# MahanFathi/iLQG-MuJoCo

Hardware: AMD Instinct MI355X
Metric: iLQR iterations/sec (FD+backward+forward) for Hopper H=500 at 1/2/4/8 GPUs (higher is better)
Workload: dtype f64

## Files before the change

### ilqg-mujoco_amd/csrc/device/dcoop_impl.h

```cpp
using namespace dev;

struct Team {
  real* w;
  int* iw;
  real* c;
  int* ci;
  int tid, nt;
};

#define TSYNC() team_sync()

#ifdef ILQG_STAMPS
#define STAMP_N 60
#define STAMP_NG 64
static __device__ unsigned long long g_stamp_acc[STAMP_NG];
static __device__ unsigned long long g_stamp_cnt[STAMP_NG];
static __device__ unsigned long long g_newton_iters;
static __device__ unsigned long long g_newton_calls;
static __device__ unsigned long long g_ls[8];
__shared__ unsigned long long s_cnt[10];
__device__ __forceinline__ void cnt_add_g(unsigned long long* g, unsigned long long v) {
  if (v) __hip_atomic_fetch_add(g, v, __ATOMIC_RELAXED, __HIP_MEMORY_SCOPE_AGENT);
}
__device__ __forceinline__ void cnt_flush() {
// ... 3350 lines not shown
        for (int i = 0; i < 3; i++) qpos[pa + i] += dt * qvel[va + i];
        pa += 3;
        va += 3;
      }
      real q[4], v[3];
      ldm<4>(q, qpos + pa);
      ldm<3>(v, qvel + va);
      quat_integrate(q, v, dt);
      for (int k = 0; k < 4; k++) qpos[pa + k] = q[k];
    } else {
      qpos[pa] += dt * qvel[va];
    }
  }
  TSYNC();
}

__device__ inline void reset_data(const auto& m, const auto& L, const Team& T) {
  real* qpos = T.w + L.qpos;
  FOR_T(i, m.nq) qpos[i] = m.qpos0[i];
  FOR_T(i, m.nv) {
    T.w[L.qvel + i] = 0;
    T.w[L.warm + i] = 0;
    T.w[L.qfrc_applied + i] = 0;
  }
  FOR_T(i, m.nu) T.w[L.ctrl + i] = 0;
  FOR_T(i, 6 * m.nbody) T.w[L.xfrc_applied + i] = 0;
  if (T.tid == 0) T.w[L.time] = 0;
  TSYNC();
}

__device__ inline int any_bad(const Team& T, const auto& C, const real* x, int n) {
  unsigned long long bad = 0;
  for (int i0 = 0; i0 < n; i0 += TEAM_SIZE) {
    const int i = i0 + T.tid;
    bad |= __ballot(i < n && is_bad(x[i]));
  }
  return bad != 0ull;
}

__device__ inline bool euler_damped(const auto& m, const Team& T) {
  const int nv = m.nv;
  unsigned long long dmask = 0;
  for (int i0 = 0; i0 < nv; i0 += TEAM_SIZE) dmask |= __ballot(i0 + T.tid < nv && m.dof_damping[i0 + T.tid] > 0);
  return dmask != 0ull;
}
__device__ inline void euler_prefactor(const auto& m, const auto& L, const auto& C, const auto& X, const Team& T) {
  const int nv = m.nv;
  real* s = T.w + L.s_euler;
  real *qH = s + nv, *qHLD = s + nv + nv * nv, *qHinv = s + nv + 2 * nv * nv;
  real* qM = T.w + L.qM;
  if (!euler_damped(m, T)) return;
  FOR_T(e, nv * nv) {
    int i = e / nv, j = e % nv;
    real v = qM[e];
    if (i == j) v += m.opt_timestep * m.dof_damping[i];
    qH[e] = v;
  }
  TSYNC();
  factor_ld(m, X, T, qH, qHLD, qHinv, T.c + C.ftmp);
}
__device__ inline void euler_finish(const auto& m, const auto& L, const auto& C, const auto& X, const Team& T,
                                    bool factored) {
  const int nv = m.nv;
  real* s = T.w + L.s_euler;
  real *qacc = s, *qHLD = s + nv + nv * nv, *qHinv = s + nv + 2 * nv * nv;
  real* qM = T.w + L.qM;
  real* dq = T.w + L.qacc;
  real* qvel = T.w + L.qvel;
  if (!euler_damped(m, T)) {
    FOR_T(i, nv) qacc[i] = dq[i];
    TSYNC();
  } else {
    FOR_T(i, nv) qacc[i] = tdot(qM + i * nv, dq, nv);
    TSYNC();
    if (!factored) euler_prefactor(m, L, C, X, T);
    solve_ld(m, X, T, qHLD, qHinv, qacc);
  }
  const real h = m.opt_timestep;
  FOR_T(i, nv) qvel[i] += qacc[i] * h;
  TSYNC();
  integrate_pos(m, T, T.w + L.qpos, qvel, h);
  if (T.tid == 0) T.w[L.time] += h;
  TSYNC();
}
__device__ inline void euler(const auto& m, const auto& L, const auto& C, const auto& X, const Team& T) {
  euler_finish(m, L, C, X, T, false);
}

#ifndef ILQG_EULER_U
#define ILQG_EULER_U 1
#endif
template <class MT>
constexpr bool euler_regs_ok() {
  if constexpr (StaticModel<MT> && ILQG_EULER_U) {
    if constexpr (MT::nv <= RMAX && MT::nq == MT::nv) {
      for (int j = 0; j < MT::njnt; j++)
        if (MT::jnt_type[j] != JNT_SLIDE && MT::jnt_type[j] != JNT_HINGE) return false;
      return true;
    }
  }
  return false;
}
template <class MT>
__device__ inline bool euler_finish_u(const auto& m, const auto& L, const auto& X, const Team& T) {
  constexpr int NV = MT::nv;
  using XT = std::remove_cvref_t<decltype(X)>;
  (void)X;
  if (!euler_damped(m, T)) return false;
  const real* s = T.w + L.s_euler;
  const real *qHLD = s + NV + NV * NV, *qHinv = s + NV + 2 * NV * NV;
  const real* qM = T.w + L.qM;
  real qa[NV], x[NV], qv[NV], qp[NV], dinv[NV], LDr[NV][NV];
  ldu(qa, T.w + L.qacc);
  ldu(qv, T.w + L.qvel);
  ldu(qp, T.w + L.qpos);
  ldu(dinv, qHinv);
  sfor<0, NV>(SLAM(ii) {
    constexpr int i = SK(ii);
    sfor<0, i>(SLAM(jj) {
      constexpr int j = SK(jj);
      if constexpr ((XT::pmask[i] >> j) & 1) LDr[i][j] = qHLD[i * NV + j];
    });
  });
  const int r = T.tid < NV ? T.tid : 0;
  real Mr[NV];
  sfor<0, NV>(SLAM(jj) { Mr[SK(jj)] = qM[r * NV + SK(jj)]; });
  gatheru(x, dotu(Mr, qa));
  sfor<0, NV>(SLAM(ii) {
    constexpr int i = NV - 1 - SK(ii);
    const bool nz = x[i] != 0;
    sfor<0, i>(SLAM(jj) {
      constexpr int j = SK(jj);
      if constexpr ((XT::pmask[i] >> j) & 1) {
        const real u = x[j] - LDr[i][j] * x[i];
        x[j] = nz ? u : x[j];
      }
    });
  });
  sfor<0, NV>(SLAM(ii) { x[SK(ii)] *= dinv[SK(ii)]; });
  sfor<0, NV>(SLAM(ii) {
    constexpr int i = SK(ii);
    sfor<0, i>(SLAM(jj) {
      constexpr int j = i - 1 - SK(jj);
      if constexpr ((XT::pmask[i] >> j) & 1) x[i] -= LDr[i][j] * x[j];
    });
  });
  const real h = m.opt_timestep;
  sfor<0, NV>(SLAM(ii) { qv[SK(ii)] += x[SK(ii)] * h; });
  sfor<0, MT::njnt>(SLAM(jj) {
    constexpr int j = SK(jj);
    constexpr int pa = MT::jnt_qposadr[j], va = MT::jnt_dofadr[j];
    qp[pa] += h * qv[va];
  });
  real* sw = T.w + L.s_euler;
  real* qvel = T.w + L.qvel;
  real* qpos = T.w + L.qpos;
  real xv = x[0], vv = qv[0], pv = qp[0];
  sfor<1, NV>(SLAM(ii) {
    xv = T.tid == SK(ii) ? x[SK(ii)] : xv;
    vv = T.tid == SK(ii) ? qv[SK(ii)] : vv;
    pv = T.tid == SK(ii) ? qp[SK(ii)] : pv;
  });
  if (T.tid < NV) {
    sw[T.tid] = xv;
    qvel[T.tid] = vv;
    qpos[T.tid] = pv;
  }
  if (T.tid == 0) T.w[L.time] += h;
  TSYNC();
  return true;
}

__device__ inline void rk4(const auto& m, const auto& L, const auto& C, const auto& X, const Team& T,
                           int maxiter, real tol) {
  const real A[9] = {0.5, 0, 0, 0, 0.5, 0, 0, 0, 1};
  const real Bw[4] = {1.0 / 6, 1.0 / 3, 1.0 / 3, 1.0 / 6};
  const int nv = m.nv, nq = m.nq, N = 4;
  const real h = m.opt_timestep;
  real* qpos = T.w + L.qpos;
  real* qvel = T.w + L.qvel;
  real* qaccw = T.w + L.qacc;
  const real time = T.w[L.time];
  real Cc[3], Tt[3];
  real* s = T.w + L.s_rk4;
  real *dX = s, *X0 = s + 2 * nv, *F = s + 2 * nv + 4 * (nq + nv);
  for (int i = 1; i < N; i++) {
    Cc[i - 1] = 0;
    for (int j = 0; j < i; j++) Cc[i - 1] += A[(i - 1) * (N - 1) + j];
    Tt[i - 1] = time + Cc[i - 1] * h;
  }
  FOR_T(k, nq) X0[k] = qpos[k];
  FOR_T(k, nv) { X0[nq + k] = qvel[k]; F[k] = qaccw[k]; }
  TSYNC();
  for (int i = 1; i < N; i++) {
    real* Xi = X0 + i * (nq + nv);
    FOR_T(k, nv) {
      real a0 = 0, a1 = 0;
      for (int j = 0; j < i; j++) {
        real a = A[(i - 1) * (N - 1) + j];
        a0 += X0[j * (nq + nv) + nq + k] * a;
        a1 += F[j * nv + k] * a;
      }
      dX[k] = a0;
      dX[nv + k] = a1;
    }
    FOR_T(k, nq + nv) Xi[k] = X0[k];
    TSYNC();
    integrate_pos(m, T, Xi, dX, h);
    FOR_T(k, nv) Xi[nq + k] += dX[nv + k] * h;
    TSYNC();
    FOR_T(k, nq) qpos[k] = Xi[k];
    FOR_T(k, nv) qvel[k] = Xi[nq + k];
    if (T.tid == 0) T.w[L.time] = Tt[i - 1];
    TSYNC();
    forward_skip(m, L, C, X, T, STAGE_NONE, maxiter, tol);
    FOR_T(k, nv) F[i * nv + k] = qaccw[k];
    TSYNC();
  }
  FOR_T(k, nv) {
    real a0 = 0, a1 = 0;
    for (int j = 0; j < N; j++) {
      a0 += X0[j * (nq + nv) + nq + k] * Bw[j];
      a1 += F[j * nv + k] * Bw[j];
    }
    dX[k] = a0;
    dX[nv + k] = a1;
  }
  TSYNC();
  FOR_T(k, nq) qpos[k] = X0[k];
  FOR_T(k, nv) qvel[k] = X0[nq + k] + dX[nv + k] * h;
  if (T.tid == 0) T.w[L.time] = time;
  TSYNC();
  integrate_pos(m, T, qpos, dX, h);
  if (T.tid == 0) T.w[L.time] += h;
  TSYNC();
}

__device__ inline void step(const auto& m, const auto& L, const auto& C, const auto& X,
                            const Team& T) {
  if (any_bad(T, C, T.w + L.qpos, m.nq)) reset_data(m, L, T);
  if (any_bad(T, C, T.w + L.qvel, m.nv)) reset_data(m, L, T);
  forward_skip(m, L, C, X, T, STAGE_NONE, m.opt_iterations, m.opt_tolerance);
  if (any_bad(T, C, T.w + L.qacc, m.nv)) {
    reset_data(m, L, T);
    forward_skip(m, L, C, X, T, STAGE_NONE, m.opt_iterations, m.opt_tolerance);
  }
  STAMP(-1);
  if (m.opt_integrator == 1)
    rk4(m, L, C, X, T, m.opt_iterations, m.opt_tolerance);
  else
    euler(m, L, C, X, T);
  STAMP(9);
}

__device__ inline void factor_m_and_euler(const auto& m, const auto& L, const auto& C, const auto& X,
                                          const Team& T, bool eul) {
  const int nv = m.nv;
  real* qM = T.w + L.qM;
  if (!(eul && euler_damped(m, T))) {
    factor_ld(m, X, T, qM, T.w + L.qLD, T.w + L.qLDinv, T.c + C.ftmp);
    return;
  }
  if (!(nv <= RMAX && has_pmask(X))) {
    factor_ld(m, X, T, qM, T.w + L.qLD, T.w + L.qLDinv, T.c + C.ftmp);
    euler_prefactor(m, L, C, X, T);
    return;
  }
  real* s = T.w + L.s_euler;
  real *qH = s + nv, *qHLD = s + nv + nv * nv, *qHinv = s + nv + 2 * nv * nv;
  using MT = std::remove_cvref_t<decltype(m)>;
  if constexpr (fld_lanes_ok<MT>()) {
    constexpr int NV = MT::nv;
    real add[NV];
    sfor<0, NV>(SLAM(ii) { add[SK(ii)] = m.opt_timestep * m.dof_damping[SK(ii)]; });
#ifdef ILQG_ASM_MARK
    asm volatile(";;MARK_F2_BEGIN" ::: "memory");
#endif
    factor_ld_lanes<std::remove_cvref_t<decltype(X)>, NV>(T.tid, qM, add, true, T.w + L.qLD, T.w + L.qLDinv,
                                                          (int)(qHLD - (T.w + L.qLD)), (int)(qHinv - (T.w + L.qLDinv)));
#ifdef ILQG_ASM_MARK
    asm volatile(";;MARK_F2_END" ::: "memory");
#endif
    return;
  }
  FOR_T(e, nv * nv) {
    int i = e / nv, j = e % nv;
    real v = qM[e];
    if (i == j) v += m.opt_timestep * m.dof_damping[i];
    qH[e] = v;
  }
  TSYNC();
#ifdef ILQG_ASM_MARK
  asm volatile(";;MARK_F2_BEGIN" ::: "memory");
#endif
  factor_ld_rows2(nv, X.pmask, T.tid, qM, T.w + L.qLD, T.w + L.qLDinv, qH, qHLD, qHinv);
#ifdef ILQG_ASM_MARK
  asm volatile(";;MARK_F2_END" ::: "memory");
#endif
}

#ifndef ILQG_FACC
#define ILQG_FACC 1
#endif
template <class MT>
__device__ inline bool factor_acc_u(const auto& m, const auto& L, const auto& X, const Team& T, bool eul) {
  constexpr int NV = MT::nv, NB = MT::nbody;
  using XT = std::remove_cvref_t<decltype(X)>;
  (void)X;
  const real* xf = T.w + L.xfrc_applied;
  static_assert(6 * NB <= TEAM_SIZE, "one ballot over xfrc_applied");
  if (__ballot(T.tid >= 6 && T.tid < 6 * NB && xf[T.tid] != 0) != 0ull) return false;
  const bool two = eul && euler_damped(m, T);
  const bool l1 = two && T.tid == 1;
  const real *qp = T.w + L.qfrc_passive, *qb = T.w + L.qfrc_bias, *qap = T.w + L.qfrc_applied;
  const real* qa = T.w + L.qfrc_act;
  const real* qM = T.w + L.qM;
  real v[NV], a[NV][NV];
  sfor<0, NV>(SLAM(jj) {
    constexpr int j = SK(jj);
    real t = qp[j] - qb[j];
    t += qap[j];
    t += qa[j];
    v[j] = t;
  });
  sfor<0, NV>(SLAM(ii) {
    constexpr int i = SK(ii);
    sfor<0, i + 1>(SLAM(jj) { a[i][SK(jj)] = qM[i * NV + SK(jj)]; });
    const real s_ = a[i][i] + m.opt_timestep * m.dof_damping[i];
    a[i][i] = l1 ? s_ : a[i][i];
  });
  sfor<0, NV>(SLAM(kk) {
    constexpr int k = NV - 1 - SK(kk);
    real dk = a[k][k];
    if (dk < MINVAL) dk = MINVAL;
    a[k][k] = dk;
    sfor<0, k>(SLAM(ii) {
      constexpr int i = k - 1 - SK(ii);
      if constexpr ((XT::pmask[k] >> i) & 1) {
        const real tmp = a[k][i] / dk;
        sfor<0, i + 1>(SLAM(jj) {
          constexpr int j = i - SK(jj);
          if constexpr (j == i || ((XT::pmask[i] >> j) & 1)) a[i][j] -= tmp * a[k][j];
        });
        a[k][i] = tmp;
      }
    });
  });
  real dinv[NV];
  sfor<0, NV>(SLAM(ii) { dinv[SK(ii)] = 1 / a[SK(ii)][SK(ii)]; });
  real x[NV];
  sfor<0, NV>(SLAM(jj) { x[SK(jj)] = v[SK(jj)]; });
  sfor<0, NV>(SLAM(ii) {
    constexpr int i = NV - 1 - SK(ii);
    const bool nz = x[i] != 0;
    sfor<0, i>(SLAM(jj) {
      constexpr int j = SK(jj);
      if constexpr ((XT::pmask[i] >> j) & 1) {
        const real u = x[j] - a[i][j] * x[i];
        x[j] = nz ? u : x[j];
      }
    });
  });
  sfor<0, NV>(SLAM(ii) { x[SK(ii)] *= dinv[SK(ii)]; });
  sfor<0, NV>(SLAM(ii) {
    constexpr int i = SK(ii);
    sfor<0, i>(SLAM(jj) {
      constexpr int j = i - 1 - SK(jj);
      if constexpr ((XT::pmask[i] >> j) & 1) x[i] -= a[i][j] * x[j];
    });
  });
  if (T.tid == 0 || l1) {
    real* s_ = T.w + L.s_euler;
    real* LD = l1 ? s_ + NV + NV * NV : T.w + L.qLD;
    real* Dinv = l1 ? s_ + NV + 2 * NV * NV : T.w + L.qLDinv;
    sfor<0, NV>(SLAM(ii) {
      constexpr int i = SK(ii);
      sfor<0, NV>(SLAM(jj) {
        constexpr int j = SK(jj);
        if constexpr (j <= i) LD[i * NV + j] = a[i][j];
        else LD[i * NV + j] = (real)0;
      });
      Dinv[i] = dinv[i];
    });
  }
  if (T.tid == 0) {
    sfor<0, NV>(SLAM(ii) {
      T.w[L.qfrc_smooth + SK(ii)] = v[SK(ii)];
      T.w[L.qacc_smooth + SK(ii)] = x[SK(ii)];
    });
  }
  TSYNC();
  return true;
}

__device__ inline bool factor_m_signal(const auto& m, const auto& L, const auto& C, const auto& X, const Team& T,
                                       bool eul, int* fm, int sid) {
  const int nv = m.nv;
  if (!(nv <= RMAX && has_pmask(X))) {
    factor_m_and_euler(m, L, C, X, T, eul);
    wave_signal(fm, sid);
    return false;
  }
  factor_ld_rows(nv, X.pmask, T.tid, T.w + L.qM, T.w + L.qLD, T.w + L.qLDinv);
  wave_signal(fm, sid);
  return eul && euler_damped(m, T);
}
__device__ inline void euler_factor_rows(const auto& m, const auto& L, const auto& X, const Team& T) {
  const int nv = m.nv;
  const real* qM = T.w + L.qM;
  real* s = T.w + L.s_euler;
  real *qH = s + nv, *qHLD = s + nv + nv * nv, *qHinv = s + nv + 2 * nv * nv;
  FOR_T(e, nv * nv) {
    int i = e / nv, j = e % nv;
    real v = qM[e];
    if (i == j) v += m.opt_timestep * m.dof_damping[i];
    qH[e] = v;
  }
  TSYNC();
  factor_ld_rows(nv, X.pmask, T.tid, qH, qHLD, qHinv);
}

#ifndef ILQG_ACC_P4
#define ILQG_ACC_P4 0
#endif
#ifndef ILQG_COLL_SPLIT
#define ILQG_COLL_SPLIT 1
#endif
#ifndef ILQG_SPLIT3
#define ILQG_SPLIT3 1
#endif
template <class MT, class XT>
constexpr unsigned long long plane_pair_mask() {
  unsigned long long mk = 0;
  for (int p = 0; p < XT::npair && p < 64; p++)
    if (MT::geom_type[XT::pair[2 * p]] == GEOM_PLANE || MT::geom_type[XT::pair[2 * p + 1]] == GEOM_PLANE)
      mk |= 1ull << p;
  return mk;
}
template <class MT, class XT>
constexpr bool coll_split_ok() {
  if constexpr (StaticModel<MT> && ILQG_COLL_SPLIT) {
    if constexpr (XT::npair > 0 && XT::npair <= 64) {
      constexpr unsigned long long pm = plane_pair_mask<MT, XT>();
      constexpr unsigned long long all = XT::npair == 64 ? ~0ull : (1ull << XT::npair) - 1;
      return pm != 0 && pm != all;
    }
  }
  return false;
}

#ifndef ILQG_PHASE_LDS
#define ILQG_PHASE_LDS 1
#endif
__device__ __forceinline__ void phase_sync() {
#if ILQG_PHASE_LDS
  __builtin_amdgcn_fence(__ATOMIC_RELEASE, "workgroup", "local");
  __builtin_amdgcn_s_barrier();
  __builtin_amdgcn_fence(__ATOMIC_ACQUIRE, "workgroup", "local");
#else
  __syncthreads();
#endif
}

__device__ inline void step_dual_split(const auto& m, const auto& L, const auto& C, const auto& X, const Team& T,
                                       int wave, int sid, auto&& pre, auto&& late) {
  const bool A = wave == 0, B = wave == 1;
  int* fq = T.ci + C.ibc + 6;
  int* ff = T.ci + C.ibc + 7;
  const bool eul = m.opt_integrator != 1;
  STAMP(-1);
  STAMPB(-1);
  STAMPC(-1);
  const bool bad = any_bad(T, C, T.w + L.qpos, m.nq) || any_bad(T, C, T.w + L.qvel, m.nv);
  if (bad) {
    if (B) {
      pre();
      late();
    }
    phase_sync();
    if (A) reset_data(m, L, T);
    phase_sync();
  }
  int* nlim_sh = T.ci + C.ibc + 5;
  constexpr bool ksplit = kin_split_ok<std::remove_cvref_t<decltype(m)>>();
  if (A) {
    if constexpr (ksplit) kinematics_primary(m, L, C, T, fq, ff, sid);
    else kinematics(m, L, C, T);
    STAMP(0);
  } else if (!B) {
    const int nl = limit_rows_pre(m, L, C, T);
    if (T.tid == 0) *nlim_sh = nl;
    passive_forces(m, L, T);
    if constexpr (ksplit) kinematics_frames(m, L, T, fq, ff, sid);
    STAMPC(48);
  } else {
    if (!bad) pre();
    STAMPB(41);
    transmission(m, L, T);
    TSYNC();
    actuator_force(m, L, T);
    STAMPB(42);
  }
  phase_sync();
  const int nlim = *nlim_sh;
  STAMP(24);
  STAMPB(32);
  STAMPC(49);
  if (A) {
    using MT = std::remove_cvref_t<decltype(m)>;
    if constexpr (StaticModel<MT> && ILQG_COM_U) com_pos_u<MT>(m, L, T);
    else com_pos(m, L, T);
    STAMP(1);
  } else {
    using MT = std::remove_cvref_t<decltype(m)>;
    using XT = std::remove_cvref_t<decltype(X)>;
    if constexpr (coll_split_ok<MT, XT>()) {
      int* fc = T.ci + C.ibc + 4;
      constexpr unsigned long long pm = plane_pair_mask<MT, XT>();
      const bool mine = T.tid < XT::npair && (((pm >> T.tid) & 1ull) != 0) == B;
      if (mine) collision_pair(m, L, C, X, T, T.tid);
      if (!B) {
        wave_signal(fc, sid);
        STAMPC(50);
      } else {
        wave_wait(fc, sid);
        collision_finish(m, L, C, X, T);
        STAMPB(33);
      }
    } else if (B) {
      collision(m, L, C, X, T);
      STAMPB(33);
    }
  }
  phase_sync();
  STAMP(25);
  STAMPB(34);
  STAMPC(51);
  bool rows_done = false;
  using MT3 = std::remove_cvref_t<decltype(m)>;
  constexpr bool split3 = ILQG_SPLIT3 && !ILQG_ACC_P4 && StaticModel<MT3> && ILQG_VEL_H && vel_regs_ok<MT3>() &&
                          euler_regs_ok<MT3>();
  if (A) {
    using MT = std::remove_cvref_t<decltype(m)>;
    if constexpr (StaticModel<MT> && ILQG_COM_U) crb_u<MT>(m, L, C, X, T);
    else crb(m, L, C, X, T);
    STAMP(2);
  } else if (B) {
    mc_contact_jac(m, L, X, T);
    TSYNC();
    const bool par = mc_alloc(m, L, C, T);
    TSYNC();
    if (!par || nlim < 0) {
      mc_rows(m, L, C, T, 0, T.iw[L.nefc]);
      TSYNC();
      rows_done = true;
    }
    if constexpr (split3) {
      if (!rows_done) {
        mc_rows(m, L, C, T, nlim, T.iw[L.nefc]);
        TSYNC();
        rows_done = true;
      }
      STAMPB(35);
      constraint_ref(m, L, T);
      TSYNC();
      STAMPB(37);
    } else {
      STAMPB(35);
    }
  } else {
    if constexpr (split3) {
      fwd_velocity_h<MT3>(m, L, T);
      STAMPC(57);
    }
  }
  phase_sync();
  STAMP(26);
  STAMPB(36);
  STAMPC(52);
  const int ne5 = T.iw[L.nefc];
  const bool spec = ne5 > 0 && ne5 <= TEAM_SIZE && m.nv <= RMAX;
  using MT5 = std::remove_cvref_t<decltype(m)>;
  constexpr bool spec_h_ok = [] {
    if constexpr (StaticModel<MT5>) return ILQG_SPEC_H && split3 && MT5::nv <= RMAX && MT5::opt_iterations < SPEC_DONE;
    else return false;
  }();
  const bool spec_h = spec_h_ok && spec;
  using MT4 = std::remove_cvref_t<decltype(m)>;
  constexpr bool acc4 = ILQG_ACC_P4 && vel_regs_ok<MT4>() && euler_regs_ok<MT4>();
  int* fm = T.ci + C.ibc + 3;
  bool acc_done = false;
  bool euler_late = false;
  if (A) {
    using MT = std::remove_cvref_t<decltype(m)>;
    if constexpr (split3) {
      if constexpr (ILQG_FACC) acc_done = factor_acc_u<MT>(m, L, X, T, eul);
      if (!acc_done) {
        factor_m_and_euler(m, L, C, X, T, eul);
        STAMP(3);
        acc_done = fwd_acceleration_u<MT>(m, L, X, T);
      }
      STAMP(7);
    } else {
      if constexpr (vel_regs_ok<MT>() && ILQG_VEL_H) fwd_velocity_h<MT>(m, L, T);
      else if constexpr (vel_regs_ok<MT>()) fwd_velocity_u<MT>(m, L, T);
      else fwd_velocity(m, L, C, T, 1);
      STAMP(6);
      if constexpr (acc4) {
        wave_wait(fm, sid);
        acc_done = fwd_acceleration_u<MT>(m, L, X, T);
        STAMP(7);
      }
    }
  } else if (B) {
    if constexpr (!split3) {
      if (!rows_done) {
        mc_rows(m, L, C, T, nlim, T.iw[L.nefc]);
        TSYNC();
      }
      constraint_ref(m, L, T);
      TSYNC();
      STAMPB(37);
    }
    if (spec) {
      using MT = std::remove_cvref_t<decltype(m)>;
      bool done_u = false;
      if constexpr (StaticModel<MT>) {
        if constexpr (ILQG_WARM_U && MT::nv <= RMAX) {
          newton_warm_prep_u<MT::nv>(m, L, C, T);
          done_u = true;
        }
      }
      if (!done_u) newton_warm_prep(m, L, C, T);
    }
    STAMPB(30);
  } else {
    if constexpr (acc4) euler_late = factor_m_signal(m, L, C, X, T, eul, fm, sid);
    else if constexpr (!split3) factor_m_and_euler(m, L, C, X, T, eul);
    STAMPC(53);
  }
  phase_sync();
  STAMP(27);
  STAMPB(39);
  STAMPC(54);
  if (A) {
    using MT = std::remove_cvref_t<decltype(m)>;
    if constexpr (!acc4 && !split3 && vel_regs_ok<MT>() && euler_regs_ok<MT>())
      acc_done = fwd_acceleration_u<MT>(m, L, X, T);
    if (!acc_done) fwd_acceleration(m, L, X, T, true);
    if constexpr (!split3) STAMP(7);
    if (spec) {
      fwd_constraint_fast(m, L, C, X, T, m.opt_iterations, m.opt_tolerance, true, spec_h ? sid : 0);
    } else {
      phase_sync();
      fwd_constraint(m, L, C, X, T, m.opt_iterations, m.opt_tolerance);
    }
    STAMP(8);
  } else {
    if (!spec_h) phase_sync();
    if (B && !bad) late();
    if (!B && euler_late) euler_factor_rows(m, L, X, T);
    if constexpr (spec_h_ok) {
      if (!B && spec_h) newton_spec_helper<MT5::nv>(L, C, T, sid);
    }
    STAMPB(38);
  }
  phase_sync();
  STAMP(29);
  STAMPB(43);
  STAMPC(55);
  if (A) {
    bool reset = false;
    if (any_bad(T, C, T.w + L.qacc, m.nv)) {
      reset = true;
      reset_data(m, L, T);
      forward_skip(m, L, C, X, T, STAGE_NONE, m.opt_iterations, m.opt_tolerance);
    }
    if (!eul) {
      rk4(m, L, C, X, T, m.opt_iterations, m.opt_tolerance);
    } else {
      bool done = false;
      using MT = std::remove_cvref_t<decltype(m)>;
      if constexpr (euler_regs_ok<MT>())
        if (!reset) done = euler_finish_u<MT>(m, L, X, T);
      if (!done) euler_finish(m, L, C, X, T, !reset);
    }
    STAMP(9);
  }
  phase_sync();
  STAMP(28);
  STAMPB(40);
  STAMPC(56);
}

__device__ inline void step_dual(const auto& m, const auto& L, const auto& C, const auto& X, const Team& T,
                                 int wave, auto&& pre, auto&& late) {
  const bool A = wave == 0;
  const bool eul = m.opt_integrator != 1;
  STAMP(-1);
  STAMPB(-1);
  const bool bad = any_bad(T, C, T.w + L.qpos, m.nq) || any_bad(T, C, T.w + L.qvel, m.nv);
  if (bad) {
    if (!A) pre();
    phase_sync();
    if (A) reset_data(m, L, T);
  }
  if (A) {
    kinematics(m, L, C, T);
    STAMP(0);
  } else if (!bad) {
    pre();
    STAMPB(41);
  }
  phase_sync();
  STAMP(24);
  STAMPB(32);
  if (A) {
    com_pos(m, L, T);
    STAMP(1);
  } else {
    collision(m, L, C, X, T);
    STAMPB(33);
  }
  phase_sync();
  STAMP(25);
  STAMPB(34);
  if (A) {
    transmission(m, L, T);
    crb(m, L, C, X, T);
    STAMP(2);
  } else {
    make_constraint(m, L, C, X, T);
    STAMPB(35);
  }
  phase_sync();
  STAMP(26);
  STAMPB(36);
  if (A) {
    fwd_velocity(m, L, C, T, 1);
    STAMP(6);
  } else {
    fwd_velocity(m, L, C, T, 2);
    STAMPB(37);
    factor_ld(m, X, T, T.w + L.qM, T.w + L.qLD, T.w + L.qLDinv, T.c + C.ftmp);
    STAMPB(42);
  }
  phase_sync();
  STAMP(27);
  STAMPB(39);
  const int ne5 = T.iw[L.nefc];
  const bool spec = ne5 > 0 && ne5 <= TEAM_SIZE && m.nv <= RMAX;
  const bool mid_sync = spec || !ILQG_EULER_EARLY;
  if (A) {
    fwd_acceleration(m, L, X, T);
    STAMP(7);
    if (spec) {
      fwd_constraint_fast(m, L, C, X, T, m.opt_iterations, m.opt_tolerance, true);
    } else {
      if (mid_sync) phase_sync();
      fwd_constraint(m, L, C, X, T, m.opt_iterations, m.opt_tolerance);
    }
    STAMP(8);
  } else {
    if (spec) {
      using MT = std::remove_cvref_t<decltype(m)>;
      bool done_u = false;
      if constexpr (StaticModel<MT>) {
        if constexpr (ILQG_WARM_U && MT::nv <= RMAX) {
          newton_warm_prep_u<MT::nv>(m, L, C, T);
          done_u = true;
        }
      }
      if (!done_u) newton_warm_prep(m, L, C, T);
    }
    STAMPB(30);
    if (mid_sync) phase_sync();
    if (eul) euler_prefactor(m, L, C, X, T);
    late();
    STAMPB(38);
  }
  phase_sync();
  STAMP(29);
  STAMPB(43);
  if (A) {
    bool reset = false;
    if (any_bad(T, C, T.w + L.qacc, m.nv)) {
      reset = true;
      reset_data(m, L, T);
      forward_skip(m, L, C, X, T, STAGE_NONE, m.opt_iterations, m.opt_tolerance);
    }
    if (!eul) rk4(m, L, C, X, T, m.opt_iterations, m.opt_tolerance);
    else euler_finish(m, L, C, X, T, !reset);
    STAMP(9);
  }
  phase_sync();
  STAMP(28);
  STAMPB(40);
}
```

### ilqg-mujoco_amd/csrc/device/rollout_body.h

```cpp
#pragma once
#ifndef ILQG_LS_NE
#define ILQG_LS_NE 0
#endif
#ifndef ILQG_LS_U
#define ILQG_LS_U 1
#endif
#ifndef ILQG_LS_TREE
#define ILQG_LS_TREE 0
#endif
#include "coop_common.h"

namespace ilqg {

struct RollArgs {
  int S, A, P;
  TrajDev nominal, out;
  int out_is_cand;
  const double *K, *k, *alphas;
  TrajDev dinit;
  const double *qfrc_applied, *xfrc_applied;
  int passive;
  CostDev cost;
  double* cost_cand;
  hipStream_t st;
  RollChunk ch;
  int cstride;
};
hipError_t launch_rollout_sch_static(const DevModel& m, const coop::CoopLayout& C, const RollArgs& a, bool lim,
                                     bool& done);
hipError_t launch_rollout_sch_generic(const DevModel& m, const WsLayout& L, const coop::CoopLayout& C,
                                      const coop::CoopAux& X, const RollArgs& a, bool lim, bool nv27, size_t lds_d);

namespace {

__device__ inline void rollout_body(const auto& m, const auto& L, const auto& C, const auto& X, const Team& T,
                                int S, int A, int P, TrajDev nom, TrajDev out, int out_is_cand, const double* K, const double* k, const double* alphas, TrajDev dinit, const double* qfrc_applied, const double* xfrc_applied, int passive, CostDev cost, double* cost_cand, RollChunk ch, int wave, auto split, auto lowreg, auto clamp, auto sched, int cstride = 0) {
  const bool prim = wave <= 0;
  STAMP_INIT();
#ifdef ILQG_STAMPS
  unsigned long long rt0 = __builtin_amdgcn_s_memrealtime(), mt0 = __builtin_amdgcn_s_memtime();
#endif
  const int lane = blockIdx.x;
  const int s = lane / A, a = lane % A;
  const int nq = m.nq, nv = m.nv, nu = m.nu, nx = 2 * nv;
  const int nhi = ch.n_hi >= 0 ? ch.n_hi : P - 1, nlo = ch.n_hi >= 0 ? ch.n_lo : 0;
  const bool resume = nhi < P - 1;
  if (resume) load_state(m, L, T, ch.carry, lane, s, qfrc_applied, xfrc_applied);
  else load_state(m, L, T, dinit, s, s, qfrc_applied, xfrc_applied);
  constexpr bool SCH = decltype(sched)::value;
  const CostDev cl = stage_cost(m, C, T, [&] {
    if constexpr (SCH) return cost_at(cost, nhi, cstride);
    else return cost;
  }());
  double* qpos = T.w + L.qpos;
  double* qvel = T.w + L.qvel;
  double* ctrl = T.w + L.ctrl;
  double* warm = T.w + L.warm;
  double* dx = T.w + L.s_fd;
  double* rec = T.c + C.rec;
  const int R = nq + nv + nu + nu * nx + nu;
  double* rec2 = rec;
  if (ch.dbuf) {
    extern __shared__ double lds[];
    const size_t off = ((size_t)(L.nd + C.nd + C.imgd) * 8 + (size_t)(L.ni + C.ni) * 4 + 15) / 16 * 16;
    rec2 = reinterpret_cast<double*>(reinterpret_cast<char*>(lds) + off);
  }
  auto recp = [&](int n) -> double* { return ((nhi - n) & 1) ? rec2 : rec; };
  auto fetch = [&](size_t pn, int t) -> double {
    if (t < nq) return nom.qpos[pn * nq + t];
    t -= nq;
    if (t < nv) return nom.qvel[pn * nv + t];
    t -= nv;
    if (t < nu) return nom.ctrl[pn * nu + t];
    t -= nu;
    if (t < nu * nx) return K[pn * nu * nx + t];
    return k[pn * nu + t - nu * nx];
  };
  using MT = std::remove_cvref_t<decltype(m)>;
  constexpr int PFR = StaticModel<MT> ? 4 : (decltype(lowreg)::value ? 1 : 20);
  double pf[PFR];
  const bool pfok = R <= PFR * TEAM_SIZE;
  [[maybe_unused]] const int CN = 3 * (nq + nv + nu);
  constexpr int CPF = [] {
    if constexpr (StaticModel<MT>) return (3 * (MT::nq + MT::nv + MT::nu) + TEAM_SIZE - 1) / TEAM_SIZE;
    else return 4;
  }();
  [[maybe_unused]] const bool cpok = CN <= CPF * TEAM_SIZE;
  if (!passive) {
    FOR_T(t, R) rec[t] = fetch((size_t)s * P + nhi, t);
    TSYNC();
  }
  const double alpha = alphas ? alphas[a] : 1.0;
  const int ob = out_is_cand ? lane : s;
  const bool ctl = wave < 0 || wave == 1;
  double c = 0;
  if (resume && ctl && T.tid == 0 && cost_cand) c = cost_cand[lane];
  auto pre_step = [&](int n) {
    const double* rq = recp(n);
    const double* rv = rq + nq;
    const double* ru = rq + nq + nv;
    const double* rK = ru + nu;
    const double* rk = rK + nu * nx;
    const bool pre = !passive && n > 0 && pfok && !ch.dbuf;
    [[maybe_unused]] double cpf[CPF];
    if constexpr (SCH) {
      if (n > nlo && cpok) {
        const double* row = cost.wq + (size_t)(n - 1) * (size_t)cstride;
#pragma unroll
        for (int q = 0; q < CPF; q++) {
          const int t = T.tid + q * TEAM_SIZE;
          cpf[q] = t < CN ? row[t] : 0.0;
        }
      }
    }
    if (pre) {
      const size_t pn1 = (size_t)s * P + (n - 1);
#pragma unroll
      for (int q = 0; q < PFR; q++) {
        const int t = T.tid + q * TEAM_SIZE;
        pf[q] = t < R ? fetch(pn1, t) : 0.0;
      }
    }
    if (!passive) {
      FOR_T(j, nx) dx[j] = j < nv ? state_diff_dof(m, j, qpos, rq) : qvel[j - nv] - rv[j - nv];
      TSYNC();
      FOR_T(i, nu) {
        double t = 0;
        int j = 0;
        if constexpr (!StaticModel<MT>) {
          for (; j + 8 <= nx; j += 8) {
            double kk[8], xx[8];
#pragma unroll
            for (int q = 0; q < 8; q++) {
              kk[q] = rK[i + (j + q) * nu];
              xx[q] = dx[j + q];
            }
#pragma unroll
            for (int q = 0; q < 8; q++) t += kk[q] * xx[q];
          }
        }
        for (; j < nx; j++) t += rK[i + j * nu] * dx[j];
        double cv = (t + alpha * rk[i]) + ru[i];
        if constexpr (decltype(clamp)::value) {
          const double lo = ch.ulim[i], hi = ch.ulim[nu + i];
          cv = cv < lo ? lo : (cv > hi ? hi : cv);
        }
        ctrl[i] = cv;
      }
      TSYNC();
    }
    const size_t po = (size_t)ob * P + n;
    FOR_T(i, nq) out.qpos[po * nq + i] = qpos[i];
    FOR_T(i, nv) {
      out.qvel[po * nv + i] = qvel[i];
      out.warm[po * nv + i] = warm[i];
    }
    FOR_T(i, nu) out.ctrl[po * nu + i] = ctrl[i];
    if (T.tid == 0) {
      out.time[po] = T.w[L.time];
      c += step_cost(m, cl, qpos, qvel, ctrl);
    }
    TSYNC();
    if constexpr (SCH) {
      if (n > nlo) {
        double* cd = T.c + C.cdesc;
        if (cpok) {
#pragma unroll
          for (int q = 0; q < CPF; q++) {
            const int t = T.tid + q * TEAM_SIZE;
            if (t < CN) cd[t] = cpf[q];
          }
        } else {
          const double* row = cost.wq + (size_t)(n - 1) * (size_t)cstride;
          FOR_T(t, CN) cd[t] = row[t];
        }
        TSYNC();
      }
    }
  };
  auto park = [&](int n) {
    if (!passive && n > 0 && !ch.dbuf) {
      if (pfok) {
#pragma unroll
        for (int q = 0; q < PFR; q++) {
          const int t = T.tid + q * TEAM_SIZE;
          if (t < R) rec[t] = pf[q];
        }
      } else {
        FOR_T(t, R) rec[t] = fetch((size_t)s * P + (n - 1), t);
      }
      TSYNC();
    }
  };
  if (wave >= 0) {
    if (threadIdx.x == 0)
      T.ci[C.ibc + 1] = T.ci[C.ibc + 2] = T.ci[C.ibc + 3] = T.ci[C.ibc + 4] = T.ci[C.ibc + 6] = T.ci[C.ibc + 7] = 0;
    __syncthreads();
  }
  for (int n = nhi; n >= nlo; n--) {
    if (wave < 0) {
      pre_step(n);
      step(m, L, C, X, T);
      park(n);
    } else {
      if constexpr (decltype(split)::value) {
        step_dual_split(m, L, C, X, T, wave, P - n, [&]() { pre_step(n); }, [&]() { park(n); });
      } else {
        step_dual(
            m, L, C, X, T, wave,
            [&]() {
              pre_step(n);
              park(n);
            },
            [&]() {
              if (ch.dbuf && !passive && n > 0) {
                double* dst = recp(n - 1);
                const size_t pn1 = (size_t)s * P + (n - 1);
                for (int t0 = T.tid; t0 < R; t0 += 4 * TEAM_SIZE) {
                  double v[4];
#pragma unroll
                  for (int q = 0; q < 4; q++) {
                    const int t = t0 + q * TEAM_SIZE;
                    v[q] = t < R ? fetch(pn1, t) : 0.0;
                  }
#pragma unroll
                  for (int q = 0; q < 4; q++)
                    if (t0 + q * TEAM_SIZE < R) dst[t0 + q * TEAM_SIZE] = v[q];
                }
              }
            });
      }
    }
  }
  if (ctl && T.tid == 0 && cost_cand) cost_cand[lane] = c;
  if (nlo > 0) {
    if (wave >= 0) __syncthreads();
    if (prim) {
      FOR_T(i, nq) ch.carry.qpos[(size_t)lane * nq + i] = qpos[i];
      FOR_T(i, nv) {
        ch.carry.qvel[(size_t)lane * nv + i] = qvel[i];
        ch.carry.warm[(size_t)lane * nv + i] = warm[i];
      }
      FOR_T(i, nu) ch.carry.ctrl[(size_t)lane * nu + i] = ctrl[i];
      if (T.tid == 0) ch.carry.time[lane] = T.w[L.time];
    }
  }
#ifdef ILQG_STAMPS
  if (prim && T.tid == 0 && blockIdx.x == 0) {
    g_stamp_acc[46] += __builtin_amdgcn_s_memrealtime() - rt0;
    g_stamp_acc[47] += __builtin_amdgcn_s_memtime() - mt0;
  }
#endif
  STAMP_FLUSH();
}

template <class SM>
constexpr int rollout_waves() { return SM::nv <= RMAX ? 3 : 2; }

inline size_t rollout_lds(size_t need) {
  static long pad = -1;
  if (pad < 0) {
    const char* e = getenv("ILQG_ROLLOUT_LDS");
    pad = e ? atol(e) : 0;
  }
  return (size_t)pad > need ? (size_t)pad : need;
}

}
}
```

Measured before the change: 645.2.

## Replace phase barriers with point-to-point wave flags in split step

Swaps two block-wide phase barriers in the three-wave split physics step for targeted signal/wait flags in LDS (com_pos→others, crb→wave B, velocity bias→wave A). Waves that do not need a result can run ahead instead of stalling on a full barrier. The factorisation of the mass matrix is also reordered so wave A only waits for the bias force right before the solve. A compile-time layout check asserts that waves running ahead never touch storage another wave still uses, and the nefc read is deferred for waves that no longer sync. This risks subtle races if the range table misses some shared buffer.

```diff
diff --git a/ilqg-mujoco_amd/csrc/device/dcoop_impl.h b/ilqg-mujoco_amd/csrc/device/dcoop_impl.h
--- a/ilqg-mujoco_amd/csrc/device/dcoop_impl.h
+++ b/ilqg-mujoco_amd/csrc/device/dcoop_impl.h
@@ -3676,8 +3676,10 @@
 #ifndef ILQG_FACC
 #define ILQG_FACC 1
 #endif
-template <class MT>
-__device__ inline bool factor_acc_u(const auto& m, const auto& L, const auto& X, const Team& T, bool eul) {
+template <class MT, class BW = std::nullptr_t>
+__device__ inline bool factor_acc_u(const auto& m, const auto& L, const auto& X, const Team& T, bool eul,
+                                    BW&& bias_wait = nullptr) {
+  constexpr bool late_bias = !std::is_same_v<std::remove_cvref_t<BW>, std::nullptr_t>;
   constexpr int NV = MT::nv, NB = MT::nbody;
   using XT = std::remove_cvref_t<decltype(X)>;
   (void)X;
@@ -3690,13 +3692,16 @@
   const real* qa = T.w + L.qfrc_act;
   const real* qM = T.w + L.qM;
   real v[NV], a[NV][NV];
-  sfor<0, NV>(SLAM(jj) {
-    constexpr int j = SK(jj);
-    real t = qp[j] - qb[j];
-    t += qap[j];
-    t += qa[j];
-    v[j] = t;
-  });
+  auto form_v = [&]() __attribute__((always_inline)) {
+    sfor<0, NV>(SLAM(jj) {
+      constexpr int j = SK(jj);
+      real t = qp[j] - qb[j];
+      t += qap[j];
+      t += qa[j];
+      v[j] = t;
+    });
+  };
+  if constexpr (!late_bias) form_v();
   sfor<0, NV>(SLAM(ii) {
     constexpr int i = SK(ii);
     sfor<0, i + 1>(SLAM(jj) { a[i][SK(jj)] = qM[i * NV + SK(jj)]; });
@@ -3722,6 +3727,10 @@
   });
   real dinv[NV];
   sfor<0, NV>(SLAM(ii) { dinv[SK(ii)] = 1 / a[SK(ii)][SK(ii)]; });
+  if constexpr (late_bias) {
+    bias_wait();
+    form_v();
+  }
   real x[NV];
   sfor<0, NV>(SLAM(jj) { x[SK(jj)] = v[SK(jj)]; });
   sfor<0, NV>(SLAM(ii) {
@@ -3823,6 +3832,70 @@
   return false;
 }
 
+#ifndef ILQG_P2P_SYNC
+#define ILQG_P2P_SYNC 1
+#endif
+__shared__ int s_p2p[4];
+struct P2PRange {
+  int lo, n;
+  bool wr;
+  int flag;
+};
+template <class MT, class XT>
+constexpr bool p2p_layout_ok() {
+  constexpr MT m{};
+  constexpr WsLayout L = make_layout(m, XT::npair, true);
+  constexpr int nv = MT::nv, nb = MT::nbody, nj = MT::njnt, ng = MT::ngeom, nq = MT::nq;
+  constexpr int nc = MT::maxcon > 0 ? MT::maxcon : 1, ne = MT::maxefc > 0 ? MT::maxefc : 1;
+  constexpr int np = XT::npair > 0 ? XT::npair : 1;
+  constexpr int npc = 14 * np > 3 * nv * nc ? 14 * np : 3 * nv * nc;
+  enum { F_CP = 1, F_QM = 2, F_V = 3, F_C = 4 };
+  if (!L.split) return false;
+  const P2PRange a[] = {
+      {L.xipos, 3 * nb, false, 0}, {L.ximat, 9 * nb, false, 0}, {L.xmat, 9 * nb, false, 0},
+      {L.xanchor, 3 * nj, false, 0}, {L.xaxis, 3 * nj, false, 0},
+      {L.scom, 3 * nb, true, F_CP}, {L.cdof, 6 * nv, true, F_CP}, {L.cinert, 10 * nb, true, F_CP},
+      {L.crb, 10 * nb, true, 0}, {L.qM, nv * nv, true, F_QM},
+      {L.qLD, nv * nv, true, 0}, {L.qLDinv, nv, true, 0}, {L.s_euler, 2 * nv + 2 * nv * nv, true, 0},
+      {L.xfrc_applied, 6 * nb, false, 0}, {L.qfrc_applied, nv, false, 0}, {L.qfrc_passive, nv, false, 0},
+      {L.qfrc_act, nv, false, 0}, {L.qfrc_bias, nv, false, F_V},
+      {L.qfrc_smooth, nv, true, 0}, {L.qacc_smooth, nv, true, 0}};
+  const P2PRange b[] = {
+      {L.gxpos, 3 * ng, false, 0}, {L.gxmat, 9 * ng, false, 0}, {L.qpos, nq, false, 0}, {L.qvel, nv, false, 0},
+      {L.warm, nv, false, 0}, {L.scom, 3 * nb, false, F_CP}, {L.cdof, 6 * nv, false, F_CP},
+      {L.qM, nv * nv, false, F_QM},
+      {L.con, CON_ND * nc, true, F_C}, {L.pcon, npc, true, F_C},
+      {L.efc_J, ne * nv, true, 0}, {L.efc_pos, ne, true, 0}, {L.efc_margin, ne, true, 0}, {L.efc_D, ne, true, 0},
+      {L.efc_KBIP, L.kstr * ne, true, 0},
+      {L.s_newton, 4 * nv + nv * nv + 2 * ne, true, F_C}, {L.efc_b, ne, true, F_C}, {L.efc_vel, ne, true, F_C},
+      {L.efc_aref, ne, true, F_C}, {L.efc_force, ne, true, F_C}, {L.qfrc_con, nv, true, 0}};
+  const P2PRange c[] = {
+      {L.gxpos, 3 * ng, false, 0}, {L.gxmat, 9 * ng, false, 0}, {L.pcon, 14 * np, true, F_C},
+      {L.qvel, nv, false, 0}, {L.cdof, 6 * nv, false, F_CP}, {L.cinert, 10 * nb, false, F_CP},
+      {L.cvel, 6 * nb, true, 0}, {L.s_con, 10 * nv, true, 0}, {L.cdof_dot, 6 * nv, true, 0},
+      {L.s_rne, 12 * nb, true, 0}, {L.qfrc_bias, nv, true, F_V}};
+  auto clash = [](const P2PRange& x, const P2PRange& y) {
+    const bool meet = x.lo < y.lo + y.n && y.lo < x.lo + x.n;
+    return meet && (x.wr || y.wr) && !(x.flag && x.flag == y.flag);
+  };
+  auto clash_any = [&](const auto& xs, const auto& ys) {
+    for (const P2PRange& x : xs)
+      for (const P2PRange& y : ys)
+        if (clash(x, y)) return true;
+    return false;
+  };
+  if (clash_any(a, b) || clash_any(a, c) || clash_any(b, c)) return false;
+  const int u0 = L.con, u1 = L.nd;
+  for (const P2PRange& x : a)
+    if (x.lo < u1 && u0 < x.lo + x.n) return false;
+  for (const P2PRange& x : c)
+    if (x.flag != F_C && x.lo < u1 && u0 < x.lo + x.n) return false;
+  for (const P2PRange& x : a) if (x.lo < 0 || x.lo + x.n > L.nd) return false;
+  for (const P2PRange& x : b) if (x.lo < 0 || x.lo + x.n > L.nd) return false;
+  for (const P2PRange& x : c) if (x.lo < 0 || x.lo + x.n > L.nd) return false;
+  return true;
+}
+
 #ifndef ILQG_PHASE_LDS
 #define ILQG_PHASE_LDS 1
 #endif
@@ -3842,6 +3915,21 @@
   int* fq = T.ci + C.ibc + 6;
   int* ff = T.ci + C.ibc + 7;
   const bool eul = m.opt_integrator != 1;
+  using MT3 = std::remove_cvref_t<decltype(m)>;
+  constexpr bool split3 = ILQG_SPLIT3 && !ILQG_ACC_P4 && StaticModel<MT3> && ILQG_VEL_H && vel_regs_ok<MT3>() &&
+                          euler_regs_ok<MT3>();
+  constexpr bool p2p = [] {
+    if constexpr (ILQG_P2P_SYNC && split3) {
+      static_assert(p2p_layout_ok<MT3, std::remove_cvref_t<decltype(X)>>(),
+                    "a wave running ahead would touch storage another wave still uses");
+      return true;
+    }
+    return false;
+  }();
+  int* fcp = s_p2p + 0;
+  int* fqm = s_p2p + 1;
+  int* fv = s_p2p + 2;
+  (void)fcp, (void)fqm, (void)fv;
   STAMP(-1);
   STAMPB(-1);
   STAMPC(-1);
@@ -3885,6 +3973,7 @@
     if constexpr (StaticModel<MT> && ILQG_COM_U) com_pos_u<MT>(m, L, T);
     else com_pos(m, L, T);
     STAMP(1);
+    if constexpr (p2p) wave_signal(fcp, sid);
   } else {
     using MT = std::remove_cvref_t<decltype(m)>;
     using XT = std::remove_cvref_t<decltype(X)>;
@@ -3906,19 +3995,21 @@
       STAMPB(33);
     }
   }
-  phase_sync();
+  if constexpr (p2p) {
+    if (!A) wave_wait(fcp, sid);
+  } else {
+    phase_sync();
+  }
   STAMP(25);
   STAMPB(34);
   STAMPC(51);
   bool rows_done = false;
-  using MT3 = std::remove_cvref_t<decltype(m)>;
-  constexpr bool split3 = ILQG_SPLIT3 && !ILQG_ACC_P4 && StaticModel<MT3> && ILQG_VEL_H && vel_regs_ok<MT3>() &&
-                          euler_regs_ok<MT3>();
   if (A) {
     using MT = std::remove_cvref_t<decltype(m)>;
     if constexpr (StaticModel<MT> && ILQG_COM_U) crb_u<MT>(m, L, C, X, T);
     else crb(m, L, C, X, T);
     STAMP(2);
+    if constexpr (p2p) wave_signal(fqm, sid);
   } else if (B) {
     mc_contact_jac(m, L, X, T);
     TSYNC();
@@ -3946,20 +4037,25 @@
     if constexpr (split3) {
       fwd_velocity_h<MT3>(m, L, T);
       STAMPC(57);
-    }
-  }
-  phase_sync();
+      if constexpr (p2p) wave_signal(fv, sid);
+    }
+  }
+  if constexpr (p2p) {
+    if (B) wave_wait(fqm, sid);
+  } else {
+    phase_sync();
+  }
   STAMP(26);
   STAMPB(36);
   STAMPC(52);
-  const int ne5 = T.iw[L.nefc];
-  const bool spec = ne5 > 0 && ne5 <= TEAM_SIZE && m.nv <= RMAX;
+  int ne5 = (!p2p || B) ? T.iw[L.nefc] : 0;
+  bool spec = ne5 > 0 && ne5 <= TEAM_SIZE && m.nv <= RMAX;
   using MT5 = std::remove_cvref_t<decltype(m)>;
   constexpr bool spec_h_ok = [] {
     if constexpr (StaticModel<MT5>) return ILQG_SPEC_H && split3 && MT5::nv <= RMAX && MT5::opt_iterations < SPEC_DONE;
     else return false;
   }();
-  const bool spec_h = spec_h_ok && spec;
+  bool spec_h = spec_h_ok && spec;
   using MT4 = std::remove_cvref_t<decltype(m)>;
   constexpr bool acc4 = ILQG_ACC_P4 && vel_regs_ok<MT4>() && euler_regs_ok<MT4>();
   int* fm = T.ci + C.ibc + 3;
@@ -3968,11 +4064,25 @@
   if (A) {
     using MT = std::remove_cvref_t<decltype(m)>;
     if constexpr (split3) {
-      if constexpr (ILQG_FACC) acc_done = factor_acc_u<MT>(m, L, X, T, eul);
-      if (!acc_done) {
-        factor_m_and_euler(m, L, C, X, T, eul);
-        STAMP(3);
-        acc_done = fwd_acceleration_u<MT>(m, L, X, T);
+      if constexpr (p2p) {
+        auto bias_wait = [&]() __attribute__((always_inline)) {
+          STAMP(3);
+          wave_wait(fv, sid);
+          STAMP(58);
+        };
+        if constexpr (ILQG_FACC) acc_done = factor_acc_u<MT>(m, L, X, T, eul, bias_wait);
+        if (!acc_done) {
+          factor_m_and_euler(m, L, C, X, T, eul);
+          bias_wait();
+          acc_done = fwd_acceleration_u<MT>(m, L, X, T);
+        }
+      } else {
+        if constexpr (ILQG_FACC) acc_done = factor_acc_u<MT>(m, L, X, T, eul);
+        if (!acc_done) {
+          factor_m_and_euler(m, L, C, X, T, eul);
+          STAMP(3);
+          acc_done = fwd_acceleration_u<MT>(m, L, X, T);
+        }
       }
       STAMP(7);
     } else {
@@ -4014,6 +4124,13 @@
     STAMPC(53);
   }
   phase_sync();
+  if constexpr (p2p) {
+    if (!B) {
+      ne5 = T.iw[L.nefc];
+      spec = ne5 > 0 && ne5 <= TEAM_SIZE && m.nv <= RMAX;
+      spec_h = spec_h_ok && spec;
+    }
+  }
   STAMP(27);
   STAMPB(39);
   STAMPC(54);
diff --git a/ilqg-mujoco_amd/csrc/device/rollout_body.h b/ilqg-mujoco_amd/csrc/device/rollout_body.h
--- a/ilqg-mujoco_amd/csrc/device/rollout_body.h
+++ b/ilqg-mujoco_amd/csrc/device/rollout_body.h
@@ -195,6 +195,8 @@
   if (wave >= 0) {
     if (threadIdx.x == 0)
       T.ci[C.ibc + 1] = T.ci[C.ibc + 2] = T.ci[C.ibc + 3] = T.ci[C.ibc + 4] = T.ci[C.ibc + 6] = T.ci[C.ibc + 7] = 0;
+    if constexpr (decltype(split)::value)
+      if (threadIdx.x == 0) coop::s_p2p[0] = coop::s_p2p[1] = coop::s_p2p[2] = 0;
     __syncthreads();
   }
   for (int n = nhi; n >= nlo; n--) {
```

Result: no change. 649.4, median of 6 (+0.7%).
